# yjh0410/YOLO-Nano

Measured on AMD Instinct MI355X. Metric: images/sec YOLO-Nano-1.0x 416x416 bs=32 inference (network + decode + NMS + host delivery), higher is better.
Workload: dtype f32 (split-f16 MFMA x3, fp32 accumulate); 1 GPU; YOLO-Nano-1.0x 416x416 bs=32/GPU fp32 inference, COCO 80-class head + NMS (BASELINE configs[1]); inputs resident in HBM, kept detections delivered to pinned host memory inside the timed region; global_batch=32, parallelism=image-sharded x1, no collective, rccl_ranks=1, launch_mode=eager, streams_per_gpu=4

## Files before the change

yolo-nano_amd/csrc/kernels_pipe.hip:

```cpp
#include "yn_internal.h"
#include "yn_device.h"

#include <cstdlib>
#include <type_traits>

namespace ynk {

typedef _Float16 ph16;
typedef _Float16 ph16x8 __attribute__((ext_vector_type(8)));
typedef _Float16 ph16x4 __attribute__((ext_vector_type(4)));

template <int BF, bool LAST, int NW>
__global__ __launch_bounds__(64 * NW, 2) void unit_pipe_kernel(ChainArgs a, int tiles, float inv_w, float inv_h)
{
    constexpr int WN = BF <= 64 ? 2 : (BF <= 128 ? 4 : 8), WM = NW / WN, NT = 1, BM = 32 * WM, NTHR = 64 * NW;
    constexpr bool STREAM = BF > 128;
    constexpr int bf = BF, KQ = (BF + 7) >> 3, PS = plane_stride(BF), S = (KQ + 1) >> 1, SMAX = S;
    constexpr int VEC = BF % 4 == 0 ? 4 : 2, CG = BF / VEC, RUN = VEC == 4 ? 4 : 8;
    constexpr unsigned ROWB = BF * 4u;
    constexpr int X1C = (int)((ROWB + 15u) / 16u), X1S = X1C * 4;
    typedef typename VecT<VEC>::type vec;
    constexpr bool RELU = true;
    static_assert(BF % 2 == 0 && BF <= 256 && WM >= 1 && WM * WN == NW && (VEC == 4 || !STREAM), "channel pairs at least, one 32-column tile per wavefront");
    extern __shared__ __attribute__((aligned(16))) unsigned char up_smem[];
    const int W = a.W, H = a.H, HW = H * W;
    constexpr bool last = LAST;
    constexpr int out_ld = LAST ? 2 * BF : BF;
    const unsigned win_bytes = (unsigned)(BM + 2 * W + 2) * ROWB;
    const unsigned win_lds = (win_bytes + 8u + 15u) & ~15u;
    unsigned char* win = up_smem;
    float* x1s = reinterpret_cast<float*>(up_smem + win_lds);
    ph16* Ph = reinterpret_cast<ph16*>(up_smem + win_lds + (unsigned)BM * X1S * 4u);
    ph16* Pl = Ph + BM * PS;
    int* mtab = reinterpret_cast<int*>(Pl + BM * PS);
    float* taps = reinterpret_cast<float*>(mtab + BM);
    const unsigned lds_win = (unsigned)(size_t)(__attribute__((address_space(3))) unsigned char*)up_smem;
    const unsigned lds_x1 = lds_win + win_lds;

    const int t = threadIdx.x, lane = t & 63, wave = __builtin_amdgcn_readfirstlane(t >> 6), l31 = lane & 31, h = lane >> 5;
    const int wm = wave % WM, wn = wave / WM;
#ifdef YN_EXP_TIMING
    const long long T_start = __builtin_readcyclecounter();
#endif
    const int TX = (tiles + 7) >> 3, jstep = (int)(gridDim.x >> 3);
    const int tend = ((int)(blockIdx.x & 7u) + 1) * TX < tiles ? ((int)(blockIdx.x & 7u) + 1) * TX : tiles;
    int tile = (int)(blockIdx.x & 7u) * TX + (int)(blockIdx.x >> 3);
    if (tile >= tend) return;

    const int t1_lim = ((a.M * (int)ROWB + 15) & ~15) - 16;
    auto win_lead = [&](int tl) { return ROWB % 16u == 0 ? 0 : (((tl * BM - W - 1) * (int)ROWB) & 15); };
    auto issue_window = [&](int tl) {
        int tt = t;
        asm volatile("" : "+v"(tt));
        const int g0 = (tl * BM - W - 1) * (int)ROWB;
        const int sh = ROWB % 16u == 0 ? 0 : (g0 & 15);
        const int gs = g0 - sh + tt * 16;
        const int nch = (int)((win_bytes + (unsigned)sh + 15u) >> 4);
        for (int c0 = 0; c0 < nch; c0 += NTHR) {
            int src = gs + c0 * 16;
            src = src < 0 ? 0 : (src > t1_lim ? t1_lim : src);
            if (c0 + tt < nch) dma16(a.t1, (unsigned)src, lds_win + (unsigned)(c0 + wave * 64) * 16u);
        }
    };
    auto issue_x1 = [&](int tl) {
        int tt = t;
        asm volatile("" : "+v"(tt));
        const int m0 = tl * BM;
        constexpr int nch = BM * X1C;
#pragma unroll
        for (int c0 = 0; c0 < nch; c0 += NTHR) {
            const int c = c0 + tt;
            const int row = c / X1C;
            const int j = c - row * X1C;
            const int m = m0 + row < a.M ? m0 + row : a.M - 1;
            const unsigned src = ((unsigned)m * (unsigned)a.x1_ld + (unsigned)a.x1_off) * 4u + (unsigned)j * 16u;
            if (c < nch) dma16(a.x1, src, lds_x1 + (unsigned)(c0 + wave * 64) * 16u);
        }
    };
    issue_window(tile);
    issue_x1(tile);

    constexpr int TAPQ = (10 * (BF / 2) + NTHR - 1) / NTHR;
    float2 tapv[TAPQ];
#pragma unroll
    for (int q = 0; q < TAPQ; ++q) {
        const int i = t + q * NTHR;
        const int ic = i < 10 * (BF / 2) ? i : 0;
        const int k = ic / (BF / 2), c2 = ic - k * (BF / 2);
        tapv[q] = *reinterpret_cast<const float2*>((k < 9 ? a.wdw + k * bf : a.bdw) + 2 * c2);
    }
    ph16x8 bw2[SMAX][NT][2], bw1[STREAM ? 1 : SMAX][NT][2];
    auto load_step = [&](const void* Wh_, const void* Wl_, int s, ph16x8 (&dst)[NT][2]) {
        const char* Wh = reinterpret_cast<const char*>(Wh_);
        const char* Wl = reinterpret_cast<const char*>(Wl_);
        const int kq = s * 2 + h < KQ ? s * 2 + h : KQ - 1;
#pragma unroll
        for (int nt = 0; nt < NT; ++nt) {
            const int n = wn * NT * 32 + nt * 32 + l31;
            const unsigned off = ((unsigned)kq * (unsigned)a.Npad + (unsigned)(n < a.Npad ? n : a.Npad - 1)) * 16u;
            dst[nt][0] = *reinterpret_cast<const ph16x8*>(Wh + off);
            dst[nt][1] = *reinterpret_cast<const ph16x8*>(Wl + off);
        }
    };
    auto load_w = [&](const void* Wh, const void* Wl, ph16x8 (&dst)[SMAX][NT][2]) {
#pragma unroll
        for (int s = 0; s < SMAX; ++s) load_step(Wh, Wl, s, dst[s]);
    };
    asm volatile("; YN_PIPE_FRAG_BEGIN" ::: "memory");
    load_w(a.Ws2h, a.Ws2l, bw2);
    if constexpr (!last && !STREAM) load_w(a.Ws1h, a.Ws1l, bw1);
    asm volatile("; YN_PIPE_FRAG_END\n\ts_waitcnt vmcnt(%0)" ::"i"(SMAX * NT * 2 * ((!last && !STREAM) ? 2 : 1)) : "memory");
    float bias2[NT], bias1n[NT];
#pragma unroll
    for (int nt = 0; nt < NT; ++nt) {
        const int n = wn * NT * 32 + nt * 32 + l31;
        bias2[nt] = n < bf ? a.b2[n] : 0.0f;
        bias1n[nt] = (!last && n < bf) ? a.b1n[n] : 0.0f;
    }
    static_assert(CG * (BM / RUN) <= NTHR, "one depthwise round per tile");
    const int cq = t % CG, pl = t / CG;
    const bool worker = pl < BM / RUN;
    {
#pragma unroll
        for (int q = 0; q < TAPQ; ++q) {
            const int i = t + q * NTHR;
            if (i < 10 * (BF / 2)) *reinterpret_cast<float2*>(taps + 2 * i) = tapv[q];
        }
    }
    {
        const int padn = PS - bf;
        for (int i = t; i < BM * padn; i += NTHR) { const int r = i / padn, c2 = bf + i - r * padn; Ph[r * PS + c2] = (ph16)0.0f; Pl[r * PS + c2] = (ph16)0.0f; }
    }
    float amax = 0.0f;
    const int jhi = bf >> 1;
    f32x16 acc0[NT], acc1[NT];

    auto act1 = [&](float v, int act) { return RELU ? __builtin_fmaxf(v, 0.0f) : apply_act(v, act); };
    const unsigned lane_w = ((unsigned)h * (WN * 32u) + (unsigned)wn * 32u + (unsigned)l31) * 16u;
    auto gemm = [&](ph16x8 (&bw)[SMAX][NT][2], auto which, bool refill) {
        const char* refill_h = reinterpret_cast<const char*>(decltype(which)::value == 1 ? a.Ws1h : a.Ws2h);
        const char* refill_l = reinterpret_cast<const char*>(decltype(which)::value == 1 ? a.Ws1l : a.Ws2l);
        unsigned lw = lane_w;
        asm volatile("" : "+v"(lw));
#pragma unroll
        for (int i = 0; i < NT; ++i)
#pragma unroll
            for (int k = 0; k < 16; ++k) { acc0[i][k] = 0.0f; acc1[i][k] = 0.0f; }
        const ph16* ahp = Ph + (wm * 32 + l31) * PS + h * 8;
        const ph16* alp = Pl + (wm * 32 + l31) * PS + h * 8;
#pragma unroll
        for (int s = 0; s < SMAX; ++s) {
            const ph16x8 ah = *reinterpret_cast<const ph16x8*>(ahp + s * 16);
            const ph16x8 al = *reinterpret_cast<const ph16x8*>(alp + s * 16);
#pragma unroll
            for (int nt = 0; nt < NT; ++nt) {
                acc0[nt] = __builtin_amdgcn_mfma_f32_32x32x16_f16(ah, bw[s][nt][0], acc0[nt], 0, 0, 0);
                acc1[nt] = __builtin_amdgcn_mfma_f32_32x32x16_f16(ah, bw[s][nt][1], acc1[nt], 0, 0, 0);
                acc1[nt] = __builtin_amdgcn_mfma_f32_32x32x16_f16(al, bw[s][nt][0], acc1[nt], 0, 0, 0);
            }
            if constexpr (STREAM && decltype(which)::value != 0) {
                if (refill) {
                    const unsigned kq = (s * 2 + 1 < KQ) ? (unsigned)(s * 2 + h) : (unsigned)(s * 2 + h < KQ ? s * 2 + h : KQ - 1);
                    const unsigned off = (s * 2 + 1 < KQ) ? lw + (unsigned)s * (2u * WN * 32u * 16u) : lw - (unsigned)h * (WN * 32u * 16u) + kq * (WN * 32u * 16u);
                    bw[s][0][0] = *reinterpret_cast<const ph16x8*>(refill_h + off);
                    bw[s][0][1] = *reinterpret_cast<const ph16x8*>(refill_l + off);
                }
            }
        }
#pragma unroll
        for (int nt = 0; nt < NT; ++nt)
#pragma unroll
            for (int r = 0; r < 16; ++r) acc0[nt][r] = __builtin_fmaf(acc1[nt][r], 1.0f / 2048.0f, acc0[nt][r]);
    };
    auto panel_landed = [&]() {
        if constexpr (STREAM) {
            static_assert(!STREAM || (SMAX == 15 && NT == 1), "30 asm operands");
#define YN_P2(s) "+v"(bw2[s][0][0]), "+v"(bw2[s][0][1])
            asm volatile("" : YN_P2(0), YN_P2(1), YN_P2(2), YN_P2(3), YN_P2(4), YN_P2(5), YN_P2(6), YN_P2(7), YN_P2(8), YN_P2(9), YN_P2(10), YN_P2(11), YN_P2(12), YN_P2(13), YN_P2(SMAX - 1));
#undef YN_P2
        }
    };
    auto split2 = [&](int r, int c, float v0, float v1) {
        amax = range_track(range_track(amax, v0), v1);
        typedef _Float16 h2 __attribute__((ext_vector_type(2)));
        h2 hi, lo;
        hi[0] = (ph16)v0; hi[1] = (ph16)v1;
        lo[0] = (ph16)((v0 - (float)hi[0]) * 2048.0f); lo[1] = (ph16)((v1 - (float)hi[1]) * 2048.0f);
        *reinterpret_cast<h2*>(Ph + r * PS + c) = hi;
        *reinterpret_cast<h2*>(Pl + r * PS + c) = lo;
    };

    auto write_mtab = [&](int tl) {
        int tq = threadIdx.x;
        asm volatile("" : "+v"(tq));
        if (tq < BM) {
            const int t = tq;
            const int m0 = tl * BM;
            const int rem0 = m0 % HW;
            const int y0 = rem0 / W, x0 = rem0 - y0 * W;
            const int q = x0 + t;
            const int dy = (int)(((float)q + 0.5f) * inv_w);
            const int x = q - dy * W;
            const int yy = y0 + dy;
            const int y = yy - (int)(((float)yy + 0.5f) * inv_h) * H;
            const int yb = (y >= 1 ? 1 : 0) | 2 | (y + 1 < H ? 4 : 0), xb = (x >= 1 ? 1 : 0) | 2 | (x + 1 < W ? 4 : 0);
            int bits = 0;
#pragma unroll
            for (int ky = 0; ky < 3; ++ky)
                if ((yb >> ky) & 1) bits |= xb << (3 * ky);
            mtab[t] = m0 + t < a.M ? bits : 0;
        }
    };
    write_mtab(tile);
#ifdef YN_EXP_TIMING
    const long long T_loop = __builtin_readcyclecounter();
    long long TS[12]; int tsn = 0, titer = 0;
#define YN_TS() TS[tsn++] = __builtin_readcyclecounter()
#else
#define YN_TS()
#endif
    auto do_tile = [&](const int tile, const int next) __attribute__((always_inline)) {
#ifdef YN_EXP_TIMING
        tsn = 0;
#endif
        YN_TS();
        const int m0 = tile * BM;
        const int nrows = a.M - m0 < BM ? a.M - m0 : BM;
        YN_TS();
        lds_barrier();

        YN_TS();
        if (worker) {
            vec wd[9];
#pragma unroll
            for (int k = 0; k < 9; ++k) wd[k] = *reinterpret_cast<const vec*>(taps + k * bf + VEC * cq);
            const vec bd = *reinterpret_cast<const vec*>(taps + 9 * bf + VEC * cq);
            const int r0 = RUN * pl;
            int bits[RUN];
#pragma unroll
            for (int q = 0; q < RUN / 4; ++q) {
                const int4 b4 = *reinterpret_cast<const int4*>(mtab + r0 + 4 * q);
                bits[4 * q] = b4.x; bits[4 * q + 1] = b4.y; bits[4 * q + 2] = b4.z; bits[4 * q + 3] = b4.w;
            }
            const unsigned char* wp = win + win_lead(tile) + ((unsigned)r0 * bf + VEC * cq) * 4u;
            vec acc[RUN];
#pragma unroll
            for (int i = 0; i < RUN; ++i) acc[i] = bd;
#pragma unroll
            for (int ky = 0; ky < 3; ++ky) {
                vec row[RUN + 2];
#pragma unroll
                for (int i = 0; i < RUN + 2; ++i) row[i] = *reinterpret_cast<const vec*>(wp + (unsigned)((ky * W + i) * bf) * 4u);
#pragma unroll
                for (int i = 0; i < RUN; ++i)
#pragma unroll
                    for (int kx = 0; kx < 3; ++kx) {
                        const bool ok = (bits[i] >> (ky * 3 + kx)) & 1;
                        vec v = row[i + kx];
                        if constexpr (VEC == 4) v = make_float4(ok ? v.x : 0.0f, ok ? v.y : 0.0f, ok ? v.z : 0.0f, ok ? v.w : 0.0f);
                        else v = make_float2(ok ? v.x : 0.0f, ok ? v.y : 0.0f);
                        vfma(acc[i], v, wd[ky * 3 + kx]);
                    }
            }
#pragma unroll
            for (int i = 0; i < RUN; ++i) {
                float o[VEC];
                if constexpr (VEC == 4) { o[0] = acc[i].x; o[1] = acc[i].y; o[2] = acc[i].z; o[3] = acc[i].w; }
                else { o[0] = acc[i].x; o[1] = acc[i].y; }
                typedef _Float16 hv __attribute__((ext_vector_type(VEC)));
                hv hi, lo;
#pragma unroll
                for (int j = 0; j < VEC; ++j) {
                    asm volatile("" : "+v"(o[j]));
                    amax = range_track(amax, o[j]);
                    hi[j] = (ph16)o[j];
                    lo[j] = (ph16)((o[j] - (float)hi[j]) * 2048.0f);
                }
                *reinterpret_cast<hv*>(Ph + (r0 + i) * PS + VEC * cq) = hi;
                *reinterpret_cast<hv*>(Pl + (r0 + i) * PS + VEC * cq) = lo;
            }
        }
        YN_TS();
        lds_barrier();
        YN_TS();
        if (next >= 0) { issue_window(next); write_mtab(next); }
        YN_TS();
        if constexpr (STREAM) {
            if constexpr (last) gemm(bw2, std::integral_constant<int, 0>{}, false);
            else gemm(bw2, std::integral_constant<int, 1>{}, true);
        } else {
            gemm(bw2, std::integral_constant<int, 0>{}, false);
        }
        YN_TS();
        if constexpr (!last) lds_barrier();

        {
            const __amdgpu_buffer_rsrc_t out_rs = buf_rsrc(a.out + (size_t)m0 * out_ld);
#pragma unroll
            for (int nt = 0; nt < NT; ++nt) {
                const int n = wn * NT * 32 + nt * 32 + l31;
                const float bias = bias2[nt];
                const bool to_global = n < (last ? bf : jhi);
                const bool to_plane = !last && n >= jhi && n < bf;
                const float* xr = x1s + (wm * 32 + 4 * h) * X1S + (n < bf ? n : 0);
#pragma unroll
                for (int g8 = 0; g8 < 4; ++g8) {
                    if (wm * 32 + 8 * g8 < nrows) {
                        float y[4], xv[4];
#pragma unroll
                        for (int q = 0; q < 4; ++q) xv[q] = xr[(q + 8 * g8) * X1S];
#pragma unroll
                        for (int q = 0; q < 4; ++q) y[q] = act1(acc0[nt][4 * g8 + q] + bias, a.act2);
                        if (to_global) {
#pragma unroll
                            for (int q = 0; q < 4; ++q) {
                                const int row = wm * 32 + q + 8 * g8 + 4 * h;
                                buf_store_b64<0>(out_rs, (unsigned)(row * out_ld + 2 * n) * 4u, make_float2(xv[q], y[q]));
                            }
                        }
                        if (to_plane) {
#pragma unroll
                            for (int q = 0; q < 4; ++q) split2(wm * 32 + q + 8 * g8 + 4 * h, 2 * (n - jhi), xv[q], y[q]);
                        }
                    }
                }
            }
        }
        YN_TS();
        lds_barrier();
        if (next >= 0) issue_x1(next);
        YN_TS();
        if constexpr (!last) {
            if constexpr (STREAM) gemm(bw2, std::integral_constant<int, 2>{}, next >= 0);
            else gemm(bw1, std::integral_constant<int, 0>{}, false);
            YN_TS();
            vm_drain();
            panel_landed();
            YN_TS();
            GemmArgs e{};
            e.out = a.t1n; e.out_ld = bf; e.out_off = 0; e.M = m0 + nrows; e.N = bf; e.Npad = a.Npad; e.bias = a.b1n; e.act = a.act1n; e.pass = nullptr;
            gemm_epilogue<NT>(e, acc0, m0 + wm * 32, wn * NT * 32, VEC == 4, lane, bias1n);
        } else {
            vm_drain();
        }
#ifdef YN_EXP_TIMING
        YN_TS();
        if (!last && t == 0 && (blockIdx.x % 61) == 5)
            printf("pipe bf %d blk %d iter %d: top %lld wait1 %lld dw %lld bar2 %lld issue %lld gemm1 %lld bar3+epi1 %lld bar4+x1 %lld gemm2 %lld drain %lld epi2 %lld total %lld\n", bf, (int)blockIdx.x, titer,
                   TS[1] - TS[0], TS[2] - TS[1], TS[3] - TS[2], TS[4] - TS[3], TS[5] - TS[4], TS[6] - TS[5], TS[7] - TS[6], TS[8] - TS[7], TS[9] - TS[8], TS[10] - TS[9], TS[11] - TS[10], TS[11] - TS[0]);
        ++titer;
#endif
    };
    {
        int next = tile + jstep < tend ? tile + jstep : -1;
        do_tile(tile, next);
        while (next >= 0) {
            tile = next;
            next = tile + jstep < tend ? tile + jstep : -1;
            do_tile(tile, next);
        }
    }
#undef YN_TS
    range_report(a.ovf, amax);
#ifdef YN_EXP_TIMING
    if (t == 0 && (blockIdx.x % 37) == 3)
        printf("pipewg bf %d last %d blk %d tiles %d prologue %lld total %lld start-stamp %lld\n", bf, (int)last, (int)blockIdx.x, titer, T_loop - T_start, __builtin_readcyclecounter() - T_start, T_start & 0xffffff);
#endif
}

static size_t unit_pipe_lds(int bf, int W, int BM)
{
    const size_t win = (((size_t)(BM + 2 * W + 2) * bf * 4 + 8 + 15) & ~(size_t)15), x1row = (((size_t)bf * 4 + 15) / 16) * 16;
    return win + (size_t)BM * x1row + (size_t)2 * BM * plane_stride(bf) * 2 + (size_t)BM * 4 + (size_t)10 * bf * 4;
}

bool launch_unit_pipe(const ChainArgs& a, hipStream_t s, bool dry)
{
    const int mode = a.pipe_mode == 1 ? 0 : (a.pipe_mode == 2 ? 2 : 1);
    const int min_tiles = a.bf > 128 ? 1 : 256;
    constexpr int wg_cap = 512;
    const bool last = a.Wp1n == nullptr;
    if (!mode || !a.Ws2h || (!last && !a.Ws1h)) return false;
    if (a.dw_act != 0 || a.act2 != 1 || (!last && a.act1n != 1)) return false;
    if ((a.M & 7) || a.t1_ld != a.bf || a.t1_off != 0 || ((a.x1_ld | a.x1_off) & ((a.bf & 3) ? 1 : 3)) || a.out_ld != (last ? 2 * a.bf : a.bf)) return false;
    if (a.Npad != ((a.bf + 31) & ~31)) return false;
    if (a.bf > 128 && a.Npad != 256) return false;
    if ((double)a.M * a.bf * 8.0 >= 4.0e9 || (double)a.M * a.x1_ld * 4.0 >= 4.0e9) return false;
#define YN_UP(BFv, LASTv, NWv)                                                                                           \
    {                                                                                                                    \
        constexpr int BM = 32 * (NWv / (BFv <= 64 ? 2 : (BFv <= 128 ? 4 : 8)));                                                             \
        const size_t lds = unit_pipe_lds(a.bf, a.W, BM);                                                                 \
        const int tiles = (a.M + BM - 1) / BM;                                                                           \
        if (lds <= (size_t)(NWv == 4 ? 80 : 160) * 1024) {                                                               \
            if (mode < 2 && tiles < min_tiles) return false;                                                             \
            if (dry) return true;                                                                                        \
            static unsigned long long attr = 0;                                                                          \
            if (attr_pending(attr)) { (void)hipFuncSetAttribute(reinterpret_cast<const void*>(unit_pipe_kernel<BFv, LASTv, NWv>), \
                                                   hipFuncAttributeMaxDynamicSharedMemorySize, (NWv == 4 ? 80 : 160) * 1024); }  \
            unsigned g = xcd_grid((unsigned)tiles);                                                                      \
            const unsigned cap = (unsigned)(NWv == 4 ? wg_cap : wg_cap / 2);                                             \
            if (g > cap) g = cap;                                                                                        \
            set_last_kernel_name("unit_pipe_kernel<" #BFv "," #LASTv "," #NWv ">");                                       \
            hipLaunchKernelGGL((unit_pipe_kernel<BFv, LASTv, NWv>), dim3(g), dim3(64 * NWv), lds, s, a, tiles, 1.0f / (float)a.W, 1.0f / (float)a.H); \
            return true;                                                                                                 \
        }                                                                                                                \
    }
#define YN_UPB(BFv) if (a.bf == BFv) { if (last) { YN_UP(BFv, true, 4) YN_UP(BFv, true, 8) } else { YN_UP(BFv, false, 4) YN_UP(BFv, false, 8) } return false; }
#define YN_UPW(BFv) if (a.bf == BFv) { if (last) { YN_UP(BFv, true, 8) } else { YN_UP(BFv, false, 8) } return false; }
    YN_UPW(232)
    YN_UPB(116)
    YN_UPB(58)
    YN_UPB(96)
    YN_UPB(48)
    YN_UPB(24)
#undef YN_UPB
// ... 151 lines not shown
```

yolo-nano_amd/csrc/kernels_stage.hip:

```cpp
#include "yn_internal.h"
#include "yn_device.h"

#include <cstdlib>

namespace ynk {

typedef _Float16 sh16;
typedef _Float16 sh16x8 __attribute__((ext_vector_type(8)));
typedef float sf32x4 __attribute__((ext_vector_type(4)));
typedef __attribute__((address_space(1))) unsigned gu32s;

#define YN_RLX_AGENT __ATOMIC_RELAXED, __HIP_MEMORY_SCOPE_AGENT

__device__ __forceinline__ void dma16_sc1(const void* gbase, unsigned goff, unsigned lds_dst)
{
    unsigned keep;
    asm volatile("s_mov_b32 %0, m0\n\ts_mov_b32 m0, %3\n\ts_nop 0\n\tglobal_load_lds_dwordx4 %1, %2 sc1\n\ts_mov_b32 m0, %0"
                 : "=&s"(keep)
                 : "v"(goff), "s"(gbase), "s"(lds_dst)
                 : "memory");
}
template <int BF, int NW, bool PUB_EARLY>
__global__ __launch_bounds__(64 * NW, 2) void stage_pipe_kernel(StageArgs a)
{
// ... 15 lines not shown
    float* taps = reinterpret_cast<float*>(mtab + BM);
    float* biasl = taps + 10 * BF;
    int* ctl = reinterpret_cast<int*>(biasl + 4 * BF);
    const unsigned lds_win = (unsigned)(size_t)(__attribute__((address_space(3))) unsigned char*)sp_smem;
    const unsigned lds_x1 = lds_win + win_lds;
    const unsigned lds_taps = lds_x1 + (unsigned)BM * X1S * 4u + 2u * BM * PS * 2u + BM * 4u;
    const unsigned lds_bias = lds_taps + 10u * BF * 4u;

    const int t = threadIdx.x, lane = t & 63, wave = __builtin_amdgcn_readfirstlane(t >> 6), l31 = lane & 31, h = lane >> 5;
    const int wm = wave % WM, wn = wave / WM;
    constexpr int CW = NW - 1;
    const int TX = (tiles + 7) >> 3;
    gu32s* const sync = (gu32s*)a.sync;
    gu32s* const flags = sync + STAGE_FLAGS;

    int myq = (int)(__builtin_amdgcn_s_getreg(20 | (3 << 11)) & 7u);
    bool exhausted = false;
    auto queue_n = [&](int q) { const int n = tiles - q * TX; return n < 0 ? 0 : (n > TX ? TX : n); };
    auto decode = [&](int q, int k, int nq) { const int u = k / nq; return (u << 20) | (q * TX + (k - u * nq)); };
    auto fetch_blocking = [&]() -> int {
        for (int tries = 0; tries < 8; ++tries) {
            const int nq = queue_n(myq);
            if (nq > 0) {
                int k = 0;
                if (lane == 0) k = (int)__hip_atomic_fetch_add(sync + myq * STAGE_HEAD_STRIDE, 1u, YN_RLX_AGENT);
                k = __builtin_amdgcn_readfirstlane(k);
                if (k < nunits * nq) return decode(myq, k, nq);
            }
            myq = (myq + 1) & 7;
        }
        exhausted = true;
        return -1;
    };
    int pend = 0;
    bool pend_on = false;
    auto fetch_issue = [&]() {
        pend_on = false;
        if (!exhausted && queue_n(myq) > 0) {
            if (lane == 0) pend = (int)__hip_atomic_fetch_add(sync + myq * STAGE_HEAD_STRIDE, 1u, YN_RLX_AGENT);
            pend_on = true;
        }
    };
    auto fetch_resolve = [&]() -> int {
        if (exhausted) return -1;
        if (pend_on) {
            const int k = __builtin_amdgcn_readfirstlane(pend), nq = queue_n(myq);
            if (k < nunits * nq) return decode(myq, k, nq);
            myq = (myq + 1) & 7;
        }
        return fetch_blocking();
    };
    unsigned pollv = 1u;
    auto poll_issue = [&](int item) {
        const int u = item >> 20, T = item & 0xfffff;
        int tt = T - 1 + (lane < 3 ? lane : 1);
        tt = tt < 0 ? 0 : (tt >= tiles ? tiles - 1 : tt);
        pollv = __hip_atomic_load(flags + (u - 1) * tiles + tt, YN_RLX_AGENT);
    };
    auto poll_ready = [&]() -> bool { return __builtin_amdgcn_ballot_w64(pollv != 0u) == ~0ull; };
    auto wait_ready = [&](int item) {
        if ((item >> 20) == 0) return;
        const unsigned long long t0 = wall_clock64();
        for (;;) {
            poll_issue(item);
            if (poll_ready()) return;
            __builtin_amdgcn_s_sleep(8);
            if (wall_clock64() - t0 > 200000000ull) {
                if (lane == 0) __hip_atomic_store(sync + STAGE_TIMEOUT, 1u, YN_RLX_AGENT);
                return;
            }
        }
    };

    const int t1_lim = ((a.M * (int)ROWB + 15) & ~15) - 16;
    auto issue_window = [&](int item) {
        const int tl = item & 0xfffff;
        const float* t1 = a.u[item >> 20].t1;
        int tt = t;
        asm volatile("" : "+v"(tt));
        const int gs = (tl * BM - W - 1) * (int)ROWB + tt * 16;
        const int nch = (int)((win_bytes + 15u) >> 4);
        for (int c0 = 0; c0 < nch; c0 += NTHR) {
            int src = gs + c0 * 16;
            src = src < 0 ? 0 : (src > t1_lim ? t1_lim : src);
            if (c0 + tt < nch) dma16_sc1(t1, (unsigned)src, lds_win + (unsigned)(c0 + wave * 64) * 16u);
        }
    };
    auto issue_x1 = [&](int item) {
        const int tl = item & 0xfffff;
        const float* x1 = a.u[item >> 20].x1;
        const unsigned x1_ld = (unsigned)a.u[item >> 20].x1_ld;
        int tt = t;
        asm volatile("" : "+v"(tt));
        const int m0 = tl * BM;
        constexpr int nch = BM * X1C;
#pragma unroll
        for (int c0 = 0; c0 < nch; c0 += NTHR) {
            const int c = c0 + tt;
            const int row = c / X1C;
            const int j = c - row * X1C;
            const int m = m0 + row < a.M ? m0 + row : a.M - 1;
            const unsigned src = (unsigned)m * x1_ld * 4u + (unsigned)j * 16u;
            if (c < nch) dma16_sc1(x1, src, lds_x1 + (unsigned)(c0 + wave * 64) * 16u);
        }
    };
    auto issue_taps = [&](int unit, int par) {
        const StageUnit& u = a.u[unit];
        int tt = t;
        asm volatile("" : "+v"(tt));
        constexpr int nW = 9 * BF / 4, nB = BF / 4;
#pragma unroll
        for (int c0 = 0; c0 < nW; c0 += NTHR)
            if (c0 + tt < nW) dma16(u.wdw, (unsigned)(c0 + tt) * 16u, lds_taps + (unsigned)(c0 + wave * 64) * 16u);
        if (wave == 1 % NW && lane < nB) dma16(u.bdw, (unsigned)lane * 16u, lds_taps + 9u * BF * 4u);
        if (wave == 2 % NW && lane < nB) dma16(u.b2, (unsigned)lane * 16u, lds_bias + (unsigned)(2 * par) * BF * 4u);
        if (wave == 3 % NW && lane < nB) dma16(u.b1n, (unsigned)lane * 16u, lds_bias + (unsigned)(2 * par + 1) * BF * 4u);
    };
    static_assert(BF / 4 <= 64, "one DMA instruction per bias row");

    if (wave == CW) {
        const int c = fetch_blocking();
        if (c >= 0) wait_ready(c);
        if (lane == 0) ctl[3] = c;
    }
    __syncthreads();
    int cur = __builtin_amdgcn_readfirstlane(ctl[3]);
    if (cur >= 0) {
    issue_window(cur);
    issue_x1(cur);
    issue_taps(cur >> 20, 0);

    sh16x8 bw2[S][2], bw1[S][2];
    const int ncol = wn * 32 + l31;
    const unsigned lane_w = ((unsigned)h * NPAD + (unsigned)(ncol < NPAD ? ncol : NPAD - 1)) * 16u;
    auto step_off = [&](unsigned lw, int s) {
        const unsigned kq = (unsigned)(s * 2 + h < KQ ? s * 2 + h : KQ - 1);
        return (s * 2 + 1 < KQ) ? lw + (unsigned)s * (2u * NPAD * 16u) : lw - (unsigned)h * (NPAD * 16u) + kq * (NPAD * 16u);
    };
    asm volatile("; YN_STAGE_FRAG_BEGIN" ::: "memory");
    {
        const StageUnit& u = a.u[cur >> 20];
#pragma unroll
        for (int s = 0; s < S; ++s) {
            bw2[s][0] = *reinterpret_cast<const sh16x8*>(reinterpret_cast<const char*>(u.Ws2h) + step_off(lane_w, s));
            bw2[s][1] = *reinterpret_cast<const sh16x8*>(reinterpret_cast<const char*>(u.Ws2l) + step_off(lane_w, s));
        }
#pragma unroll
        for (int s = 0; s < S; ++s) {
            bw1[s][0] = *reinterpret_cast<const sh16x8*>(reinterpret_cast<const char*>(u.Ws1h) + step_off(lane_w, s));
            bw1[s][1] = *reinterpret_cast<const sh16x8*>(reinterpret_cast<const char*>(u.Ws1l) + step_off(lane_w, s));
        }
    }
    asm volatile("; YN_STAGE_FRAG_END\n\ts_waitcnt vmcnt(%0)" ::"i"(4 * S) : "memory");
    const int cq = t % CG, pl = t / CG;
    const bool worker = pl < BM / RUN;
    {
        constexpr int padn = PS - BF;
        for (int i = t; i < BM * padn; i += NTHR) { const int r = i / padn, c2 = BF + i - r * padn; Ph[r * PS + c2] = (sh16)0.0f; Pl[r * PS + c2] = (sh16)0.0f; }
    }
    float amax = 0.0f;
    constexpr int jhi = BF >> 1;
    f32x16 acc0, acc1;
    int par = 0;

    auto gemm = [&](sh16x8 (&bw)[S][2], const void* rh_, const void* rl_, bool refill, sh16x8 (&bo)[S][2], const void* qh_, const void* ql_) {
        const char* rh = reinterpret_cast<const char*>(rh_);
        const char* rl = reinterpret_cast<const char*>(rl_);
        const char* qh = reinterpret_cast<const char*>(qh_);
        const char* ql = reinterpret_cast<const char*>(ql_);
        unsigned lw = lane_w;
        asm volatile("" : "+v"(lw));
#pragma unroll
        for (int k = 0; k < 16; ++k) { acc0[k] = 0.0f; acc1[k] = 0.0f; }
        const sh16* ahp = Ph + (wm * 32 + l31) * PS + h * 8;
        const sh16* alp = Pl + (wm * 32 + l31) * PS + h * 8;
#pragma unroll
        for (int s = 0; s < S; ++s) {
            const sh16x8 ah = *reinterpret_cast<const sh16x8*>(ahp + s * 16);
            const sh16x8 al = *reinterpret_cast<const sh16x8*>(alp + s * 16);
            acc0 = __builtin_amdgcn_mfma_f32_32x32x16_f16(ah, bw[s][0], acc0, 0, 0, 0);
            acc1 = __builtin_amdgcn_mfma_f32_32x32x16_f16(ah, bw[s][1], acc1, 0, 0, 0);
            acc1 = __builtin_amdgcn_mfma_f32_32x32x16_f16(al, bw[s][0], acc1, 0, 0, 0);
            if (refill) {
                const unsigned off = step_off(lw, s);
                bo[s][0] = *reinterpret_cast<const sh16x8*>(qh + off);
                bo[s][1] = *reinterpret_cast<const sh16x8*>(ql + off);
                bw[s][0] = *reinterpret_cast<const sh16x8*>(rh + off);
                bw[s][1] = *reinterpret_cast<const sh16x8*>(rl + off);
            }
        }
#pragma unroll
        for (int r = 0; r < 16; ++r) acc0[r] = __builtin_fmaf(acc1[r], 1.0f / 2048.0f, acc0[r]);
    };
    auto split2 = [&](int r, int c, float v0, float v1) {
        amax = range_track(range_track(amax, v0), v1);
        typedef _Float16 h2 __attribute__((ext_vector_type(2)));
        h2 hi, lo;
        hi[0] = (sh16)v0; hi[1] = (sh16)v1;
        lo[0] = (sh16)((v0 - (float)hi[0]) * 2048.0f); lo[1] = (sh16)((v1 - (float)hi[1]) * 2048.0f);
        *reinterpret_cast<h2*>(Ph + r * PS + c) = hi;
        *reinterpret_cast<h2*>(Pl + r * PS + c) = lo;
    };
    auto write_mtab = [&](int item) {
        if (t < BM) {
            const int m0 = (item & 0xfffff) * BM;
            const int rem0 = m0 % HW;
            const int y0 = rem0 / W, x0 = rem0 - y0 * W;
            const int q = x0 + t;
            const int dy = (int)(((float)q + 0.5f) * a.inv_w);
            const int x = q - dy * W;
            const int yy = y0 + dy;
            const int y = yy - (int)(((float)yy + 0.5f) * a.inv_h) * H;
            const int yb = (y >= 1 ? 1 : 0) | 2 | (y + 1 < H ? 4 : 0), xb = (x >= 1 ? 1 : 0) | 2 | (x + 1 < W ? 4 : 0);
            int bits = 0;
#pragma unroll
            for (int ky = 0; ky < 3; ++ky)
                if ((yb >> ky) & 1) bits |= xb << (3 * ky);
            mtab[t] = m0 + t < a.M ? bits : 0;
        }
    };
    write_mtab(cur);
    auto publish = [&](int item) {
        if (t == 0) __hip_atomic_store(flags + (item >> 20) * tiles + (item & 0xfffff), 1u, YN_RLX_AGENT);
    };

#ifdef YN_EXP_STAGE_TIMING
    long long* dbg = reinterpret_cast<long long*>(ctl + 16);
    if (t < 24) dbg[t] = 0;
    long long dprev = __builtin_readcyclecounter();
    const long long T_start = dprev;
#define YN_TS(i) do { if (wave == 1 % NW) { const long long now_ = __builtin_readcyclecounter(); if (lane == 0) dbg[i] += now_ - dprev; dprev = now_; } } while (0)
#define YN_CNT(i) do { if (wave == 1 % NW && lane == 0) dbg[i] += 1; } while (0)
#else
#define YN_TS(i)
#define YN_CNT(i)
#endif
    bool pub_out = false;
    auto do_tile = [&](const int cur, const int prev) __attribute__((always_inline)) -> int {
        const int unit = cur >> 20, tile = cur & 0xfffff;
        const StageUnit& U = a.u[unit];
        const int m0 = tile * BM;
        const int nrows = a.M - m0 < BM ? a.M - m0 : BM;
        YN_TS(15);
        lds_barrier();
        YN_TS(0); YN_CNT(16);

        if (worker) {
            float4 wd[9];
#pragma unroll
            for (int k = 0; k < 9; ++k) wd[k] = *reinterpret_cast<const float4*>(taps + k * BF + 4 * cq);
            const float4 bd = *reinterpret_cast<const float4*>(taps + 9 * BF + 4 * cq);
            const int r0 = RUN * pl;
            int bits[RUN];
            {
                const int4 b4 = *reinterpret_cast<const int4*>(mtab + r0);
                bits[0] = b4.x; bits[1] = b4.y; bits[2] = b4.z; bits[3] = b4.w;
            }
            const unsigned char* wp = win + ((unsigned)r0 * BF + 4 * cq) * 4u;
            float4 acc[RUN];
#pragma unroll
            for (int i = 0; i < RUN; ++i) acc[i] = bd;
#pragma unroll
            for (int ky = 0; ky < 3; ++ky) {
                float4 row[RUN + 2];
#pragma unroll
                for (int i = 0; i < RUN + 2; ++i) row[i] = *reinterpret_cast<const float4*>(wp + (unsigned)((ky * W + i) * BF) * 4u);
#pragma unroll
                for (int i = 0; i < RUN; ++i)
#pragma unroll
                    for (int kx = 0; kx < 3; ++kx) {
                        const bool ok = (bits[i] >> (ky * 3 + kx)) & 1;
                        float4 v = row[i + kx];
                        v = make_float4(ok ? v.x : 0.0f, ok ? v.y : 0.0f, ok ? v.z : 0.0f, ok ? v.w : 0.0f);
                        vfma(acc[i], v, wd[ky * 3 + kx]);
                    }
            }
#pragma unroll
            for (int i = 0; i < RUN; ++i) {
                float o[4] = {acc[i].x, acc[i].y, acc[i].z, acc[i].w};
                typedef _Float16 hv __attribute__((ext_vector_type(4)));
                hv hi, lo;
#pragma unroll
                for (int j = 0; j < 4; ++j) {
                    asm volatile("" : "+v"(o[j]));
                    amax = range_track(amax, o[j]);
                    hi[j] = (sh16)o[j];
                    lo[j] = (sh16)((o[j] - (float)hi[j]) * 2048.0f);
                }
                *reinterpret_cast<hv*>(Ph + (r0 + i) * PS + 4 * cq) = hi;
                *reinterpret_cast<hv*>(Pl + (r0 + i) * PS + 4 * cq) = lo;
            }
        }
        YN_TS(1);
        if (!PUB_EARLY && prev >= 0) vm_drain();
        lds_barrier();
        YN_TS(2);
        if (!PUB_EARLY && prev >= 0) publish(prev);
        if (wave == CW) fetch_issue();
        YN_TS(3);
        gemm(bw2, nullptr, nullptr, false, bw1, nullptr, nullptr);
        YN_TS(4);
        lds_barrier();
        YN_TS(5);
        if (wave == CW) {
            const int n = fetch_resolve();
            if (n >= 0 && (n >> 20) > 0) poll_issue(n); else pollv = 1u;
            if (lane == 0) ctl[0] = n;
        }

        {
            const __amdgpu_buffer_rsrc_t ro = buf_rsrc(U.out);
            const int n = ncol;
            const float bias = n < BF ? biasl[(2 * par) * BF + n] : 0.0f;
            const bool to_global = n < jhi;
            const bool to_plane = n >= jhi && n < BF;
            const float* xr = x1s + (wm * 32 + 4 * h) * X1S + (n < BF ? n : 0);
#pragma unroll
            for (int g8 = 0; g8 < 4; ++g8) {
                if (wm * 32 + 8 * g8 < nrows) {
                    float y[4], xv[4];
#pragma unroll
                    for (int q = 0; q < 4; ++q) xv[q] = xr[(q + 8 * g8) * X1S];
#pragma unroll
                    for (int q = 0; q < 4; ++q) y[q] = __builtin_fmaxf(acc0[4 * g8 + q] + bias, 0.0f);
                    if (to_global) {
#pragma unroll
                        for (int q = 0; q < 4; ++q) {
                            const int row = m0 + wm * 32 + q + 8 * g8 + 4 * h;
                            buf_store_b64<16>(ro, (unsigned)(row * BF + 2 * n) * 4u, make_float2(xv[q], y[q]));
                        }
                    }
                    if (to_plane) {
#pragma unroll
                        for (int q = 0; q < 4; ++q) split2(wm * 32 + q + 8 * g8 + 4 * h, 2 * (n - jhi), xv[q], y[q]);
                    }
                }
            }
        }
        if (wave == CW) {
            const bool r = poll_ready();
            if (lane == 0) ctl[2] = r ? 1 : 0;
        }
        YN_TS(6);
        lds_barrier();
        YN_TS(7);
        const int nxt = __builtin_amdgcn_readfirstlane(ctl[0]);
        const bool have_next = nxt >= 0;
        const bool rdy = have_next && __builtin_amdgcn_readfirstlane(ctl[2]) != 0;
        const bool sw = have_next && (nxt >> 20) != unit;
        const StageUnit& UN = a.u[have_next ? (nxt >> 20) : unit];
        if (sw) { issue_taps(nxt >> 20, par ^ 1); YN_CNT(20); }
        if (rdy) { issue_window(nxt); write_mtab(nxt); issue_x1(nxt); YN_CNT(18); }
        YN_TS(8);
        gemm(bw1, UN.Ws1h, UN.Ws1l, sw, bw2, UN.Ws2h, UN.Ws2l);
        YN_TS(9);
        vm_drain();
        if constexpr (S == 8) {
            asm volatile("" : "+v"(bw2[0][0]), "+v"(bw2[0][1]), "+v"(bw2[1][0]), "+v"(bw2[1][1]), "+v"(bw2[2][0]), "+v"(bw2[2][1]), "+v"(bw2[3][0]), "+v"(bw2[3][1]),
                              "+v"(bw2[4][0]), "+v"(bw2[4][1]), "+v"(bw2[5][0]), "+v"(bw2[5][1]), "+v"(bw2[6][0]), "+v"(bw2[6][1]), "+v"(bw2[7][0]), "+v"(bw2[7][1]));
            asm volatile("" : "+v"(bw1[0][0]), "+v"(bw1[0][1]), "+v"(bw1[1][0]), "+v"(bw1[1][1]), "+v"(bw1[2][0]), "+v"(bw1[2][1]), "+v"(bw1[3][0]), "+v"(bw1[3][1]),
                              "+v"(bw1[4][0]), "+v"(bw1[4][1]), "+v"(bw1[5][0]), "+v"(bw1[5][1]), "+v"(bw1[6][0]), "+v"(bw1[6][1]), "+v"(bw1[7][0]), "+v"(bw1[7][1]));
        } else {
#pragma unroll
            for (int s = 0; s < S; ++s) {
                asm volatile("" : "+v"(bw2[s][0]), "+v"(bw2[s][1]), "+v"(bw1[s][0]), "+v"(bw1[s][1]));
            }
        }
        YN_TS(10);
        {
            const __amdgpu_buffer_rsrc_t rt = buf_rsrc(U.t1n);
            const float bias = ncol < BF ? biasl[(2 * par + 1) * BF + ncol] : 0.0f;
            const int j = lane & 3;
            const int nq = wn * 32 + (l31 & ~3);
#pragma unroll
            for (int g = 0; g < 4; ++g) {
                float v0 = __builtin_fmaxf(acc0[4 * g + 0] + bias, 0.0f), v1 = __builtin_fmaxf(acc0[4 * g + 1] + bias, 0.0f);
                float v2 = __builtin_fmaxf(acc0[4 * g + 2] + bias, 0.0f), v3 = __builtin_fmaxf(acc0[4 * g + 3] + bias, 0.0f);
                {
                    const float s0 = (j & 1) ? v0 : v1, s1 = (j & 1) ? v2 : v3;
                    const float r0 = quad_xor1(s0), r1 = quad_xor1(s1);
                    if (j & 1) { v0 = r0; v2 = r1; } else { v1 = r0; v3 = r1; }
                }
                {
                    const float s0 = (j & 2) ? v0 : v2, s1 = (j & 2) ? v1 : v3;
                    const float r0 = quad_xor2(s0), r1 = quad_xor2(s1);
                    if (j & 2) { v0 = r0; v1 = r1; } else { v2 = r0; v3 = r1; }
                }
                const int m = m0 + wm * 32 + 8 * g + 4 * h + j;
                if (m < m0 + nrows && nq < BF) buf_store_b128<16>(rt, (unsigned)(m * BF + nq) * 4u, make_float4(v0, v1, v2, v3));
            }
        }
        YN_TS(11);
        const bool block = have_next && !rdy;
        pub_out = PUB_EARLY || !have_next || block;
        if (pub_out) {
            vm_drain();
            lds_barrier();
            publish(cur);
        }
        YN_TS(12);
        if (block) {
            YN_CNT(19);
            if (wave == CW) wait_ready(nxt);
            lds_barrier();
            issue_window(nxt); write_mtab(nxt); issue_x1(nxt);
            vm_drain();
        }
        YN_TS(13);
        par ^= sw ? 1 : 0;
        return nxt;
    };
    {
        int nxt = do_tile(cur, -1);
        while (nxt >= 0) {
            const int prev = pub_out ? -1 : cur;
            cur = nxt;
            nxt = do_tile(cur, prev);
        }
    }
    range_report(a.ovf, amax);
#ifdef YN_EXP_STAGE_TIMING
    __syncthreads();
    if (t == 64 % NTHR && (blockIdx.x % 41) == 7)
        printf("stagewg blk %d xcc %d tiles %lld rdy %lld block %lld sw %lld | total %lld | bar1 %lld dw %lld bar2 %lld issue %lld gemm1 %lld bar3 %lld epi1 %lld bar4 %lld x1 %lld gemm2 %lld drain %lld epi2 %lld pub %lld blockwait %lld top %lld\n",
               (int)blockIdx.x, (int)(__builtin_amdgcn_s_getreg(20 | (3 << 11)) & 7u), dbg[16], dbg[18], dbg[19], dbg[20], __builtin_readcyclecounter() - T_start,
               dbg[0], dbg[1], dbg[2], dbg[3], dbg[4], dbg[5], dbg[6], dbg[7], dbg[8], dbg[9], dbg[10], dbg[11], dbg[12], dbg[13], dbg[15]);
#endif
    }
// ... 54 lines not shown
```

yolo-nano_amd/csrc/yn_device.h:

```cpp
#pragma once
#include "yn_internal.h"
#include "yn_stage_form.h"

namespace ynk {

typedef float f32x16 __attribute__((ext_vector_type(16)));

#ifdef YN_EXP_NO_RANGE
__device__ __forceinline__ float range_track(float amax, float) { return amax; }
__device__ __forceinline__ void range_report(unsigned*, float) {}
#else
__device__ __forceinline__ float range_track(float amax, float x) { return __builtin_fmaxf(amax, __builtin_fabsf(x)); }
__device__ __forceinline__ void range_report(unsigned* ovf, float amax)
{
    if (ovf && amax >= 65504.0f) atomicOr(ovf, 1u);
}
#endif

__device__ __forceinline__ float apply_act(float v, int act)
{
    const float slope = act == 2 ? 0.1f : 1.0f;
    const unsigned keep = act == 1 ? 0u : 0xffffffffu;
    const float neg = __uint_as_float(__float_as_uint(slope * v) & keep);
    return v > 0.0f ? v : neg;
// ... 103 lines not shown
typedef _Float16 c3h16x4 __attribute__((ext_vector_type(4)));

__host__ __device__ constexpr int gemm_split_smem_halves(int BM, int BN, int KC = 32) { return 2 * BM * (KC + 8) + 2 * (KC / 8) * BN * 8; }

template <int WM, int WN, int NT, int KC = 32>
__device__ __forceinline__ void gemm_split_tile(const GemmArgs& a, c3h16* smem, int m0, int n0, f32x16 (&acc0)[NT])
{
    constexpr int BM = 32 * WM, BN = 32 * NT * WN, AST = KC + 8, OQ = KC / 8;
    constexpr int A_PER = (BM * OQ + 255) / 256;
    constexpr int B_PER = (2 * OQ * BN + 255) / 256;
    c3h16* Ah = smem;
    c3h16* Al = smem + BM * AST;
    c3h16* Bh = smem + 2 * BM * AST;
    const int t = threadIdx.x, lane = t & 63, wave = t >> 6;
    const int l31 = lane & 31, h = lane >> 5;
    const int wm = wave % WM, wn = wave / WM;
    const int KQ = (a.K + 7) >> 3, nchunks = (a.K + KC - 1) / KC;
    const bool vecA = ((a.K | a.in_ld | a.in_off) & 3) == 0;
    const c3h16* Wsh = reinterpret_cast<const c3h16*>(a.Wsh);
    const c3h16* Wsl = reinterpret_cast<const c3h16*>(a.Wsl);

    float4 a_reg[A_PER][2];
    c3h16x8 b_reg[B_PER];
    float amax = 0.0f;
    auto prefetch = [&](int c) {
#pragma unroll
        for (int i = 0; i < A_PER; ++i) {
            const int g = t + 256 * i;
            const int row = g / OQ, k = c * KC + (g % OQ) * 8;
            const int m = m0 + row;
            const float* p = a.in + (size_t)(m < a.M ? m : a.M - 1) * a.in_ld + a.in_off;
            if (vecA) {
                a_reg[i][0] = *reinterpret_cast<const float4*>(p + (k < a.K ? k : 0));
                a_reg[i][1] = *reinterpret_cast<const float4*>(p + (k + 4 < a.K ? k + 4 : 0));
            } else {
                float2 v[4];
#pragma unroll
                for (int j = 0; j < 4; ++j) v[j] = *reinterpret_cast<const float2*>(p + (k + 2 * j < a.K ? k + 2 * j : 0));
                a_reg[i][0] = make_float4(v[0].x, v[0].y, v[1].x, v[1].y);
                a_reg[i][1] = make_float4(v[2].x, v[2].y, v[3].x, v[3].y);
            }
        }
#pragma unroll
        for (int i = 0; i < B_PER; ++i) {
            const int g = t + 256 * i;
            const int pl = g / (OQ * BN), r = g - pl * (OQ * BN);
            const int o = r / BN, n = r - o * BN;
            const int kq = min(c * (KC / 8) + o, KQ - 1), nn = min(n0 + n, a.Npad - 1);
            b_reg[i] = *reinterpret_cast<const c3h16x8*>(((pl & 1) ? Wsl : Wsh) + ((size_t)kq * a.Npad + nn) * 8);
        }
    };
    auto stage = [&](int c) {
#pragma unroll
        for (int i = 0; i < A_PER; ++i) {
            const int g = t + 256 * i;
            if (g < BM * OQ) {
                const int k = c * KC + (g % OQ) * 8;
                float x8[8] = {a_reg[i][0].x, a_reg[i][0].y, a_reg[i][0].z, a_reg[i][0].w, a_reg[i][1].x, a_reg[i][1].y, a_reg[i][1].z, a_reg[i][1].w};
#pragma unroll
                for (int j = 0; j < 8; ++j) x8[j] = (k + (vecA ? (j & 4) : (j & 6)) < a.K) ? x8[j] : 0.0f;
                c3h16x8 hi, lo;
#pragma unroll
                for (int j = 0; j < 8; ++j) { amax = range_track(amax, x8[j]); hi[j] = (c3h16)x8[j]; lo[j] = (c3h16)((x8[j] - (float)hi[j]) * 2048.0f); }
                *reinterpret_cast<c3h16x8*>(Ah + (g / OQ) * AST + (g % OQ) * 8) = hi;
                *reinterpret_cast<c3h16x8*>(Al + (g / OQ) * AST + (g % OQ) * 8) = lo;
            }
        }
#pragma unroll
        for (int i = 0; i < B_PER; ++i) {
            const int g = t + 256 * i;
            if (g < 2 * OQ * BN) *reinterpret_cast<c3h16x8*>(Bh + (size_t)g * 8) = b_reg[i];
        }
    };
    f32x16 acc1[NT];
#pragma unroll
    for (int i = 0; i < NT; ++i)
#pragma unroll
        for (int r = 0; r < 16; ++r) { acc0[i][r] = 0.0f; acc1[i][r] = 0.0f; }

    prefetch(0);
    stage(0);
    __syncthreads();
    for (int c = 0; c < nchunks; ++c) {
        if (c + 1 < nchunks) prefetch(c + 1);
        const c3h16* Ahb = Ah + (wm * 32 + l31) * AST + h * 8;
        const c3h16* Alb = Al + (wm * 32 + l31) * AST + h * 8;
        const c3h16* Bhb = Bh + (size_t)(h * BN + wn * NT * 32 + l31) * 8;
        const c3h16* Blb = Bhb + OQ * BN * 8;
#pragma unroll
        for (int ks = 0; ks < KC / 16; ++ks) {
            const c3h16x8 ah = *reinterpret_cast<const c3h16x8*>(Ahb + ks * 16);
            const c3h16x8 al = *reinterpret_cast<const c3h16x8*>(Alb + ks * 16);
#pragma unroll
            for (int nt = 0; nt < NT; ++nt) {
                const c3h16x8 bh = *reinterpret_cast<const c3h16x8*>(Bhb + (size_t)(ks * 2 * BN + nt * 32) * 8);
                const c3h16x8 bl = *reinterpret_cast<const c3h16x8*>(Blb + (size_t)(ks * 2 * BN + nt * 32) * 8);
                acc0[nt] = __builtin_amdgcn_mfma_f32_32x32x16_f16(ah, bh, acc0[nt], 0, 0, 0);
                acc1[nt] = __builtin_amdgcn_mfma_f32_32x32x16_f16(ah, bl, acc1[nt], 0, 0, 0);
                acc1[nt] = __builtin_amdgcn_mfma_f32_32x32x16_f16(al, bh, acc1[nt], 0, 0, 0);
            }
        }
        if (c + 1 < nchunks) {
            __syncthreads();
            stage(c + 1);
            __syncthreads();
        }
    }
#pragma unroll
    for (int nt = 0; nt < NT; ++nt)
#pragma unroll
        for (int r = 0; r < 16; ++r) acc0[nt][r] = __builtin_fmaf(acc1[nt][r], 1.0f / 2048.0f, acc0[nt][r]);
    range_report(a.ovf, amax);
}


__device__ __forceinline__ void dma16(const void* gbase, unsigned goff, unsigned lds_dst)
{
    unsigned keep;
    asm volatile("s_mov_b32 %0, m0\n\ts_mov_b32 m0, %3\n\ts_nop 0\n\tglobal_load_lds_dwordx4 %1, %2\n\ts_mov_b32 m0, %0"
                 : "=&s"(keep)
                 : "v"(goff), "s"(gbase), "s"(lds_dst)
                 : "memory");
}
__device__ __forceinline__ void lds_barrier() { asm volatile("s_waitcnt lgkmcnt(0)\n\ts_barrier" ::: "memory"); }
__device__ __forceinline__ void vm_drain() { asm volatile("s_waitcnt vmcnt(0)" ::: "memory"); }

__device__ __forceinline__ __amdgpu_buffer_rsrc_t buf_rsrc(void* p) { return __builtin_amdgcn_make_buffer_rsrc(p, 0, -1, 0x00020000); }
template <int AUX>
__device__ __forceinline__ void buf_store_b128(__amdgpu_buffer_rsrc_t r, unsigned off, float4 v)
{
    typedef float f4 __attribute__((ext_vector_type(4)));
    typedef unsigned u4 __attribute__((__vector_size__(4 * sizeof(unsigned))));
    const f4 d = {v.x, v.y, v.z, v.w};
    __builtin_amdgcn_raw_buffer_store_b128(__builtin_bit_cast(u4, d), r, (int)off, 0, AUX);
}
template <int AUX>
__device__ __forceinline__ void buf_store_b64(__amdgpu_buffer_rsrc_t r, unsigned off, float2 v)
{
    typedef float f2 __attribute__((ext_vector_type(2)));
    typedef unsigned u2 __attribute__((__vector_size__(2 * sizeof(unsigned))));
    const f2 d = {v.x, v.y};
    __builtin_amdgcn_raw_buffer_store_b64(__builtin_bit_cast(u2, d), r, (int)off, 0, AUX);
}

template <int V> struct VecT;
template <> struct VecT<2> { typedef float2 type; };
template <> struct VecT<4> { typedef float4 type; };
__device__ __forceinline__ void vfma(float2& acc, const float2 v, const float2 w) { acc.x = __builtin_fmaf(v.x, w.x, acc.x); acc.y = __builtin_fmaf(v.y, w.y, acc.y); }
__device__ __forceinline__ void vfma(float4& acc, const float4 v, const float4 w)
{
    acc.x = __builtin_fmaf(v.x, w.x, acc.x); acc.y = __builtin_fmaf(v.y, w.y, acc.y);
    acc.z = __builtin_fmaf(v.z, w.z, acc.z); acc.w = __builtin_fmaf(v.w, w.w, acc.w);
}
__device__ __forceinline__ float2 vact(float2 v, int act) { return make_float2(apply_act(v.x, act), apply_act(v.y, act)); }
__device__ __forceinline__ float4 vact(float4 v, int act) { return make_float4(apply_act(v.x, act), apply_act(v.y, act), apply_act(v.z, act), apply_act(v.w, act)); }

}
```

yolo-nano_amd/csrc/yn_stage_form.h:

```cpp
#pragma once
#include <cstddef>

namespace ynk {

constexpr int plane_stride(int C) { return ((((C + 7) >> 3) + 1) & ~1) * 8 + 8; }

constexpr int stage_pipe_bm(int bf, int nw) { return 32 * (nw / (bf <= 64 ? 2 : 4)); }

constexpr size_t stage_pipe_lds(int bf, int W, int bm)
{
    return (((size_t)(bm + 2 * W + 2) * bf * 4 + 15) & ~(size_t)15) + (size_t)bm * bf * 4 + (size_t)2 * bm * plane_stride(bf) * 2 + (size_t)bm * 4 +
           (size_t)14 * bf * 4 + 64 + 192;
}

struct StagePipeForm {
    int nw, bm;
    size_t lds, lds_max;
};

inline StagePipeForm stage_pipe_form(int bf, int W)
{
    if (bf != 24 && bf != 48 && bf != 96 && bf != 116) return {0, 0, 0, 0};
    for (int nw = 4; nw <= 8; nw += 4) {
        const int bm = stage_pipe_bm(bf, nw);
        const size_t lds = stage_pipe_lds(bf, W, bm), lds_max = (size_t)(nw == 4 ? 80 : 160) * 1024;
        if (lds <= lds_max && W + 1 <= bm) return {nw, bm, lds, lds_max};
    }
    return {0, 0, 0, 0};
}

}
```

Baseline: 49780 images/s.

## Add wave-uniform interior fast path to depthwise 3x3 and wave-aligned thread mapping

```diff
diff --git a/yolo-nano_amd/csrc/kernels_pipe.hip b/yolo-nano_amd/csrc/kernels_pipe.hip
--- a/yolo-nano_amd/csrc/kernels_pipe.hip
+++ b/yolo-nano_amd/csrc/kernels_pipe.hip
@@ -21,6 +21,7 @@
     constexpr int X1C = (int)((ROWB + 15u) / 16u), X1S = X1C * 4;
     typedef typename VecT<VEC>::type vec;
     constexpr bool RELU = true;
+    constexpr bool DW_PACK = SMAX * NT * 8 * ((!LAST && !STREAM) ? 2 : 1) < 128;
     static_assert(BF % 2 == 0 && BF <= 256 && WM >= 1 && WM * WN == NW && (VEC == 4 || !STREAM), "channel pairs at least, one 32-column tile per wavefront");
     extern __shared__ __attribute__((aligned(16))) unsigned char up_smem[];
     const int W = a.W, H = a.H, HW = H * W;
@@ -118,8 +119,9 @@
         bias1n[nt] = (!last && n < bf) ? a.b1n[n] : 0.0f;
     }
     static_assert(CG * (BM / RUN) <= NTHR, "one depthwise round per tile");
-    const int cq = t % CG, pl = t / CG;
-    const bool worker = pl < BM / RUN;
+    constexpr bool DWA = dw_wave_aligned(CG, BM / RUN, NW);
+    const int cq = DWA ? lane % CG : t % CG, pl = DWA ? wave * (BM / RUN / NW) + lane / CG : t / CG;
+    const bool worker = DWA ? lane < CG * (BM / RUN / NW) : pl < BM / RUN;
     {
 #pragma unroll
         for (int q = 0; q < TAPQ; ++q) {
@@ -246,21 +248,43 @@
             vec acc[RUN];
 #pragma unroll
             for (int i = 0; i < RUN; ++i) acc[i] = bd;
-#pragma unroll
-            for (int ky = 0; ky < 3; ++ky) {
-                vec row[RUN + 2];
-#pragma unroll
-                for (int i = 0; i < RUN + 2; ++i) row[i] = *reinterpret_cast<const vec*>(wp + (unsigned)((ky * W + i) * bf) * 4u);
-#pragma unroll
-                for (int i = 0; i < RUN; ++i)
-#pragma unroll
-                    for (int kx = 0; kx < 3; ++kx) {
-                        const bool ok = (bits[i] >> (ky * 3 + kx)) & 1;
-                        vec v = row[i + kx];
-                        if constexpr (VEC == 4) v = make_float4(ok ? v.x : 0.0f, ok ? v.y : 0.0f, ok ? v.z : 0.0f, ok ? v.w : 0.0f);
-                        else v = make_float2(ok ? v.x : 0.0f, ok ? v.y : 0.0f);
-                        vfma(acc[i], v, wd[ky * 3 + kx]);
-                    }
+            int all9 = bits[0];
+#pragma unroll
+            for (int i = 1; i < RUN; ++i) all9 &= bits[i];
+            if (__builtin_amdgcn_ballot_w64(all9 != 0x1ff) == 0) {
+                asm volatile("; YN_DW_FAST_BEGIN" ::: "memory");
+#pragma unroll
+                for (int ky = 0; ky < 3; ++ky) {
+                    vec row[RUN + 2];
+#pragma unroll
+                    for (int i = 0; i < RUN + 2; ++i) row[i] = *reinterpret_cast<const vec*>(wp + (unsigned)((ky * W + i) * bf) * 4u);
+#pragma unroll
+                    for (int i = 0; i < RUN; ++i)
+#pragma unroll
+                        for (int kx = 0; kx < 3; ++kx) {
+                            if constexpr (DW_PACK) vfma(acc[i], row[i + kx], wd[ky * 3 + kx]);
+                            else vfma_single(acc[i], row[i + kx], wd[ky * 3 + kx]);
+                        }
+                    if (ky < 2) asm volatile("" ::: "memory");
+                }
+                asm volatile("; YN_DW_FAST_END" ::: "memory");
+            } else {
+#pragma unroll
+                for (int ky = 0; ky < 3; ++ky) {
+                    vec row[RUN + 2];
+#pragma unroll
+                    for (int i = 0; i < RUN + 2; ++i) row[i] = *reinterpret_cast<const vec*>(wp + (unsigned)((ky * W + i) * bf) * 4u);
+#pragma unroll
+                    for (int i = 0; i < RUN; ++i)
+#pragma unroll
+                        for (int kx = 0; kx < 3; ++kx) {
+                            const bool ok = (bits[i] >> (ky * 3 + kx)) & 1;
+                            vec v = row[i + kx];
+                            if constexpr (VEC == 4) v = make_float4(ok ? v.x : 0.0f, ok ? v.y : 0.0f, ok ? v.z : 0.0f, ok ? v.w : 0.0f);
+                            else v = make_float2(ok ? v.x : 0.0f, ok ? v.y : 0.0f);
+                            vfma(acc[i], v, wd[ky * 3 + kx]);
+                        }
+                }
             }
 #pragma unroll
             for (int i = 0; i < RUN; ++i) {
diff --git a/yolo-nano_amd/csrc/kernels_stage.hip b/yolo-nano_amd/csrc/kernels_stage.hip
--- a/yolo-nano_amd/csrc/kernels_stage.hip
+++ b/yolo-nano_amd/csrc/kernels_stage.hip
@@ -191,8 +191,9 @@
         }
     }
     asm volatile("; YN_STAGE_FRAG_END\n\ts_waitcnt vmcnt(%0)" ::"i"(4 * S) : "memory");
-    const int cq = t % CG, pl = t / CG;
-    const bool worker = pl < BM / RUN;
+    constexpr bool DWA = dw_wave_aligned(CG, BM / RUN, NW);
+    const int cq = DWA ? lane % CG : t % CG, pl = DWA ? wave * (BM / RUN / NW) + lane / CG : t / CG;
+    const bool worker = DWA ? lane < CG * (BM / RUN / NW) : pl < BM / RUN;
     {
         constexpr int padn = PS - BF;
         for (int i = t; i < BM * padn; i += NTHR) { const int r = i / padn, c2 = BF + i - r * padn; Ph[r * PS + c2] = (sh16)0.0f; Pl[r * PS + c2] = (sh16)0.0f; }
@@ -299,20 +300,37 @@
             float4 acc[RUN];
 #pragma unroll
             for (int i = 0; i < RUN; ++i) acc[i] = bd;
-#pragma unroll
-            for (int ky = 0; ky < 3; ++ky) {
-                float4 row[RUN + 2];
-#pragma unroll
-                for (int i = 0; i < RUN + 2; ++i) row[i] = *reinterpret_cast<const float4*>(wp + (unsigned)((ky * W + i) * BF) * 4u);
-#pragma unroll
-                for (int i = 0; i < RUN; ++i)
-#pragma unroll
-                    for (int kx = 0; kx < 3; ++kx) {
-                        const bool ok = (bits[i] >> (ky * 3 + kx)) & 1;
-                        float4 v = row[i + kx];
-                        v = make_float4(ok ? v.x : 0.0f, ok ? v.y : 0.0f, ok ? v.z : 0.0f, ok ? v.w : 0.0f);
-                        vfma(acc[i], v, wd[ky * 3 + kx]);
-                    }
+            constexpr bool DW_FAST = BF > 48;
+            if (DW_FAST && __builtin_amdgcn_ballot_w64((bits[0] & bits[1] & bits[2] & bits[3]) != 0x1ff) == 0) {
+                asm volatile("; YN_DW_FAST_BEGIN" ::: "memory");
+#pragma unroll
+                for (int ky = 0; ky < 3; ++ky) {
+                    float4 row[RUN + 2];
+#pragma unroll
+                    for (int i = 0; i < RUN + 2; ++i) row[i] = *reinterpret_cast<const float4*>(wp + (unsigned)((ky * W + i) * BF) * 4u);
+#pragma unroll
+                    for (int i = 0; i < RUN; ++i)
+#pragma unroll
+                        for (int kx = 0; kx < 3; ++kx) vfma_single(acc[i], row[i + kx], wd[ky * 3 + kx]);
+                    if (ky < 2) asm volatile("" ::: "memory");
+                }
+                asm volatile("; YN_DW_FAST_END" ::: "memory");
+            } else {
+#pragma unroll
+                for (int ky = 0; ky < 3; ++ky) {
+                    float4 row[RUN + 2];
+#pragma unroll
+                    for (int i = 0; i < RUN + 2; ++i) row[i] = *reinterpret_cast<const float4*>(wp + (unsigned)((ky * W + i) * BF) * 4u);
+#pragma unroll
+                    for (int i = 0; i < RUN; ++i)
+#pragma unroll
+                        for (int kx = 0; kx < 3; ++kx) {
+                            const bool ok = (bits[i] >> (ky * 3 + kx)) & 1;
+                            float4 v = row[i + kx];
+                            v = make_float4(ok ? v.x : 0.0f, ok ? v.y : 0.0f, ok ? v.z : 0.0f, ok ? v.w : 0.0f);
+                            vfma(acc[i], v, wd[ky * 3 + kx]);
+                        }
+                }
             }
 #pragma unroll
             for (int i = 0; i < RUN; ++i) {
diff --git a/yolo-nano_amd/csrc/yn_device.h b/yolo-nano_amd/csrc/yn_device.h
--- a/yolo-nano_amd/csrc/yn_device.h
+++ b/yolo-nano_amd/csrc/yn_device.h
@@ -279,6 +279,12 @@
     acc.x = __builtin_fmaf(v.x, w.x, acc.x); acc.y = __builtin_fmaf(v.y, w.y, acc.y);
     acc.z = __builtin_fmaf(v.z, w.z, acc.z); acc.w = __builtin_fmaf(v.w, w.w, acc.w);
 }
+__device__ __forceinline__ void vfma_single(float& acc, const float v, const float w) { asm("v_fmac_f32 %0, %1, %2" : "+v"(acc) : "v"(v), "v"(w)); }
+__device__ __forceinline__ void vfma_single(float2& acc, const float2 v, const float2 w) { vfma_single(acc.x, v.x, w.x); vfma_single(acc.y, v.y, w.y); }
+__device__ __forceinline__ void vfma_single(float4& acc, const float4 v, const float4 w)
+{
+    vfma_single(acc.x, v.x, w.x); vfma_single(acc.y, v.y, w.y); vfma_single(acc.z, v.z, w.z); vfma_single(acc.w, v.w, w.w);
+}
 __device__ __forceinline__ float2 vact(float2 v, int act) { return make_float2(apply_act(v.x, act), apply_act(v.y, act)); }
 __device__ __forceinline__ float4 vact(float4 v, int act) { return make_float4(apply_act(v.x, act), apply_act(v.y, act), apply_act(v.z, act), apply_act(v.w, act)); }
 
diff --git a/yolo-nano_amd/csrc/yn_stage_form.h b/yolo-nano_amd/csrc/yn_stage_form.h
--- a/yolo-nano_amd/csrc/yn_stage_form.h
+++ b/yolo-nano_amd/csrc/yn_stage_form.h
@@ -29,4 +29,38 @@
     return {0, 0, 0, 0};
 }
 
+constexpr bool dw_wave_aligned(int cg, int runs, int nw) { return runs % nw == 0 && cg * (runs / nw) <= 64 && cg * runs > 64 * (nw - 1); }
+constexpr int dw_thread_run(int t, int cg, int runs, int nw)
+{
+    if (dw_wave_aligned(cg, runs, nw)) return (t & 63) < cg * (runs / nw) ? (t >> 6) * (runs / nw) + (t & 63) / cg : -1;
+    return t / cg < runs ? t / cg : -1;
 }
+
+struct DwInterior {
+    long long fast, waves;
+};
+
+inline DwInterior dw_interior_waves(int W, int H, int M, int BM, int RUN, int cg, int threads)
+{
+    const int runs = BM / RUN, nw = threads / 64;
+    DwInterior r = {0, 0};
+    for (int m0 = 0; m0 < M; m0 += BM)
+        for (int w = 0; w < nw; ++w) {
+            int lo = -1, hi = -1;
+            for (int l = 0; l < 64; ++l) {
+                const int run = dw_thread_run(w * 64 + l, cg, runs, nw);
+                if (run >= 0) { if (lo < 0) lo = run; hi = run; }
+            }
+            if (lo < 0) continue;
+            ++r.waves;
+            bool all9 = true;
+            for (int row = lo * RUN; row < (hi + 1) * RUN && all9; ++row) {
+                const int m = m0 + row, rem = m % (H * W), y = rem / W, x = rem - y * W;
+                all9 = m < M && x >= 1 && x + 1 < W && y >= 1 && y + 1 < H;
+            }
+            if (all9) ++r.fast;
+        }
+    return r;
+}
+
+}
```

Result: no change. 49880 images/s (median of 6 runs) (+0.2%).
